# srvk/eesen

Hardware: AMD Instinct MI355X
Metric: CTC training frames/sec (whole node), 4x512 BiLSTM (higher is better)
Workload: dtype f32

## Files before the change

### eesen_amd/csrc/net.cpp

```cpp
#include "net.h"

#include <algorithm>
#include <cmath>
#include <cstdio>
#include <cstring>

namespace eesen {


int PhaseTimer::begin(hipStream_t st, int phase) {
  if (!on_) return -1;
  if (used_ == spans_.size()) spans_.emplace_back();
  spans_[used_].phase = phase;
  spans_[used_].a.record(st);
  return (int)used_++;
}
void PhaseTimer::end(hipStream_t st, int idx) {
  if (!on_ || idx < 0) return;
  spans_[idx].b.record(st);
}
void PhaseTimer::collect(float* out, int nphase) {
  for (int i = 0; i < nphase; ++i) out[i] = 0.f;
  for (size_t i = 0; i < used_; ++i) {
    spans_[i].b.wait();
// ... 615 lines not shown
      EESEN_REQUIRE((long)L.inj_fmask.size() == (long)net.rows * ldY, EESEN_ERR_INVALID, "injected forward mask has the wrong shape");
      EESEN_HIP_CHECK(hipMemcpyAsync(L.fmask.p, L.inj_fmask.data(), L.inj_fmask.size() * sizeof(float), hipMemcpyHostToDevice, net.st));
      EESEN_HIP_CHECK(hipStreamSynchronize(net.st));
    } else {
      dropout_mask(net.st, L.fmask.p, net.rows, ldY, ldY, fwd_p, net.drop_seed + (++net.drop_counter) * 0x632BE59BD9B4E019ull, fw_seq);
    }
    L.cur_fwd_drop = true;
  }
  L.inj_fmask.clear(); L.inj_rmask.clear(); L.inj_rmask_rows = 0; L.inj_coin = -1;
}

void Net::propagate(const float* in, int nrows, int ld, bool is_device) {
  EESEN_REQUIRE(finalized, EESEN_ERR_STATE, "net not finalized");
  EESEN_REQUIRE(S > 0, EESEN_ERR_STATE, "SetSeqLengths must precede Propagate");
  EESEN_REQUIRE(nrows > 0 && nrows % S == 0, EESEN_ERR_INVALID, "row count must be a positive multiple of the sequence count");
  const int D = layers[0].din, D4 = pad4(D);
  EESEN_REQUIRE(ld >= D, EESEN_ERR_INVALID, "input leading dimension smaller than InputDim");
  EESEN_HIP_CHECK(hipSetDevice(device));
  rows = nrows;
  T = rows / S;
  for (int v : lens) EESEN_REQUIRE(v <= T, EESEN_ERR_INVALID, "sequence length exceeds the number of frames");
  timer.reset();

  if (input.reserve((size_t)rows * D4) || D4 != D) EESEN_HIP_CHECK(hipMemsetAsync(input.p, 0, (size_t)rows * D4 * sizeof(float), st));
  if (is_device) {
    EESEN_HIP_CHECK(hipMemcpy2DAsync(input.p, (size_t)D4 * sizeof(float), in, (size_t)ld * sizeof(float), (size_t)D * sizeof(float), rows,
                                     hipMemcpyDeviceToDevice, st));
  } else {
    PinBuf& hs = in_stage[in_stage_idx++ & 1];
    const size_t bytes = (size_t)rows * D * sizeof(float);
    float* staged = static_cast<float*>(hs.reserve(bytes, bytes + bytes / 4));
    for (int r = 0; r < rows; ++r) std::memcpy(staged + (size_t)r * D, in + (size_t)r * ld, (size_t)D * sizeof(float));
    EESEN_HIP_CHECK(hipMemcpy2DAsync(input.p, (size_t)D4 * sizeof(float), staged, (size_t)D * sizeof(float), (size_t)D * sizeof(float), rows,
                                     hipMemcpyHostToDevice, st));
    hs.used(st);
  }
  forward_pass();
}

Net::FwdEarly Net::fwd_early(int li, const RecPlan& fp, int T) const {
  FwdEarly E;
  const Layer& L = layers[li];
  const Layer* nxt = li + 1 < (int)layers.size() ? &layers[li + 1] : nullptr;
  const int nd = L.ndir, ldY = nd * L.H;
  const long rows = (long)T * S;
  const bool pers = fp.kind != kRecNone;
  E.gate = pers && overlap && gate_fwd && !fwd_bf16 && !L.cur_fwd_drop && fp.units <= 8 && nxt && nxt->is_lstm() && T >= 2 && rows >= 128 &&
           fp.one_window &&
           (nxt->ndir * 4 * nxt->H) % 128 == 0 && ldY % 16 == 0 && nd * fp.seq_tiles * kShards <= 64;
  E.mile_step = (3 * T) / 4;
  E.mid = pers && overlap && tn.fwd_mid && !E.gate && !L.cur_fwd_drop && fp.leaves_room && nd == 2 && nxt && nxt->is_lstm() &&
          T >= 32 && E.mile_step + 1 < T && fp.one_window;
  if (E.mid) {
    E.r0 = ((T - 1 - E.mile_step) * S + 255) / 256 * 256;
    E.r1 = (E.mile_step + 1) * S / 256 * 256;
    if (E.r1 <= E.r0) E.r0 = E.r1 = 0;
  }
  return E;
}

bool Net::fwd_quad_rule(int li, const RecPlan& fp, int T, int r0, int r1, int steps[2]) const {
  steps[0] = steps[1] = -1;
  if (!tn.fwd_quad || li < 1 || r1 <= r0 || r0 <= 0 || (long)r1 >= (long)T * S) return false;
  const Layer& L = layers[li];
  if (L.ndir != 2 || fp.kind != kRecFwdBf || !fp.fn_guard || !fp.one_window || !fp.leaves_room || (4 * L.H) % 256 != 0) return false;
  steps[0] = std::min(r0 / S, T - 1 - (r1 - 1) / S);
  steps[1] = std::min(r1 / S, T - 1 - (r0 - 1) / S);
  return steps[0] >= 2 && steps[1] >= steps[0];
}

void Net::forward_pass() {
  const float* x = input.p;
  int ldx = pad4(layers[0].din);
  ++steps_since_clean;
  info_fwd_persistent = info_lstm_layers = info_fwd_bf16 = 0;
  dg_owner[0] = dg_owner[1] = -1;
  bool g_gated = false;
  int gated_rows = 0;
  int mid_r0 = 0, mid_r1 = 0;
  const bool half = gemm_mode() == 2;
  ensure_weight_amax();
  amx_valid = half;
  for (Layer& L : layers) {
    const int li_ = (int)(&L - layers.data());
    GemmBound x_amax, w_amax;
    if (half && L.trainable()) {
      if (x_is_bounded(li_)) x_amax = bound_one();
      else { measure(x, rows, L.din, ldx, L.bx.rows, L.bx.cols); x_amax = GemmBound{L.bx.rows.p, 1}; }
      w_amax = GemmBound{L.bw.rows.p, 1};
    }
    if (L.is_lstm()) {
      const int H = L.H, nd = L.ndir, ldY = nd * H, ldG = nd * 4 * H;
      L.G.reserve((size_t)rows * ldG);
      const size_t state = (size_t)(T + 2) * S * ldY;
      L.C.reserve(state);
      L.Y.reserve(state);
      if (persistent && H % 32 == 0) L.X.reserve((size_t)T * nd * ((S + 15) / 16) * (size_t)(H / 32) * 768);
      const size_t blk = (size_t)S * ldY * sizeof(float);
      EESEN_HIP_CHECK(hipMemsetAsync(L.C.p, 0, blk, st));
      EESEN_HIP_CHECK(hipMemsetAsync(L.Y.p, 0, blk, st));
      EESEN_HIP_CHECK(hipMemsetAsync(L.C.p + (size_t)(T + 1) * S * ldY, 0, blk, st));
      EESEN_HIP_CHECK(hipMemsetAsync(L.Y.p + (size_t)(T + 1) * S * ldY, 0, blk, st));
      prepare_dropout(*this, L);
      LstmLayerDev v = lstm_view(*this, L, T);
      const RecPlan fp = persistent ? lstm_fwd_plan(v) : RecPlan{};
      const bool pers = fp.kind != kRecNone;
      int quad_steps[2];
      const bool quad = !g_gated && fwd_quad_rule(li_, fp, T, mid_r0, mid_r1, quad_steps);
      if (quad) {
        unsigned* gw = mile.p + ((li_ - 1) & 1) * kMileRegion + kGuardWord;
        const int N4 = 4 * H;
        const float* Wx = params.p + L.p_off + L.off_wx;
        const float* bias = params.p + L.p_off + L.off_bias;
        GemmBound w_hi = w_amax;
        if (w_hi.p && w_hi.per_index) w_hi.p += N4;
        const int ti_ = timer.begin(st, 0);
        gemm_f32(st, true, true, mid_r0, N4, L.din, 1.f, x, ldx, Wx, pad4(L.din), 0.f, L.G.p, ldG, bias, nullptr, 0, 0, fwd_bf16, x_amax, w_amax);
        gemm_f32(st, true, true, rows - mid_r1, N4, L.din, 1.f, x + (size_t)mid_r1 * ldx, ldx, Wx + (size_t)N4 * pad4(L.din), pad4(L.din), 0.f,
                 L.G.p + (size_t)mid_r1 * ldG + N4, ldG, bias + N4, nullptr, 0, 0, fwd_bf16, x_amax, w_hi);
        timer.end(st, ti_);
        EESEN_HIP_CHECK(hipEventRecord(ev_quad_go, st));
        EESEN_HIP_CHECK(hipMemsetD32Async(reinterpret_cast<hipDeviceptr_t>(gw), 1, 1, st2));
        EESEN_HIP_CHECK(hipStreamWaitEvent(st2, ev_quad_go, 0));
        const int late_lds = tn.fwd_quad == 2 ? 64 : (tn.side_lds_kb >= 0 ? tn.side_lds_kb : (gemm_mode() >= 1 ? 48 : 32)) * 1024;
        const int tj_ = timer.begin(st2, 0);
        gemm_f32(st2, true, true, rows - mid_r1, N4, L.din, 1.f, x + (size_t)mid_r1 * ldx, ldx, Wx, pad4(L.din), 0.f, L.G.p + (size_t)mid_r1 * ldG, ldG,
                 bias, nullptr, 0, late_lds, fwd_bf16, x_amax, w_amax);
        gemm_f32(st2, true, true, mid_r0, N4, L.din, 1.f, x, ldx, Wx + (size_t)N4 * pad4(L.din), pad4(L.din), 0.f, L.G.p + N4, ldG, bias + N4,
                 nullptr, 0, late_lds, fwd_bf16, x_amax, w_hi);
        timer.end(st2, tj_);
        EESEN_HIP_CHECK(hipMemsetD32Async(reinterpret_cast<hipDeviceptr_t>(gw + 1), 1, 1, st2));
        EESEN_HIP_CHECK(hipEventRecord(ev_quad_done, st2));
        v.guard[0] = gw; v.guard_step[0] = quad_steps[0];
        v.guard[1] = gw + 1; v.guard_step[1] = quad_steps[1];
        mid_r0 = mid_r1 = 0;
      } else if (g_gated) {
        if (gated_rows < rows) {
          const int ti_ = timer.begin(st, 0);
          gemm_f32(st, true, true, rows - gated_rows, ldG, L.din, 1.f, x + (size_t)gated_rows * ldx, ldx, params.p + L.p_off + L.off_wx,
                   pad4(L.din), 0.f, L.G.p + (size_t)gated_rows * ldG, ldG, params.p + L.p_off + L.off_bias, nullptr, 0, 0, fwd_bf16, x_amax, w_amax);
          timer.end(st, ti_);
        }
        EESEN_HIP_CHECK(hipStreamWaitEvent(st, ev_gate_done, 0));
        g_gated = false;
      } else if (mid_r1 > mid_r0) {
        const int ti_ = timer.begin(st, 0);
        const int parts[2][2] = {{0, mid_r0}, {mid_r1, rows}};
        for (const auto& pr : parts)
          if (pr[1] > pr[0])
            gemm_f32(st, true, true, pr[1] - pr[0], ldG, L.din, 1.f, x + (size_t)pr[0] * ldx, ldx, params.p + L.p_off + L.off_wx, pad4(L.din),
                     0.f, L.G.p + (size_t)pr[0] * ldG, ldG, params.p + L.p_off + L.off_bias, nullptr, 0, 0, fwd_bf16, x_amax, w_amax);
        timer.end(st, ti_);
        EESEN_HIP_CHECK(hipStreamWaitEvent(st, ev_gate_done, 0));
        mid_r0 = mid_r1 = 0;
      } else {
        const int ti_ = timer.begin(st, 0);
        gemm_f32(st, true, true, rows, ldG, L.din, 1.f, x, ldx, params.p + L.p_off + L.off_wx, pad4(L.din), 0.f, L.G.p, ldG,
                 params.p + L.p_off + L.off_bias, nullptr, 0, 0, fwd_bf16, x_amax, w_amax);
        timer.end(st, ti_);
      }
      Layer* nxt = (&L - layers.data()) + 1 < (long)layers.size() ? &layers[(&L - layers.data()) + 1] : nullptr;
      const FwdEarly early = fwd_early(li_, fp, T);
      const bool plan_gate = early.gate;
      const int mile_step = early.mile_step;
      const bool plan_mid = early.mid;
      { const int ti_ = timer.begin(st, 1);
      v.poll_delay = delay_fwd;
      v.poll_raw = poll_raw;
      if (plan_mid) {
        mile.reserve(2 * kMileRegion);
        unsigned* region = mile.p + (li_ & 1) * kMileRegion;
        EESEN_HIP_CHECK(hipMemsetAsync(region, 0, kMileRegion * sizeof(unsigned), st));
        EESEN_HIP_CHECK(hipEventRecord(ev_gate_reset, st));
        v.milestone = region;
        v.milestone_step = mile_step;
      }
      if (pers) lstm_fwd_launch(st, fp, v, ctl.p, ctl.p + kCtlWords - 1, spin_limit, trace.p, plan_gate ? ev_gate_reset.get() : nullptr);
      else
        for (int step = 0; step < T; ++step) lstm_fwd_step(st, v, step);
      info_fwd_persistent += pers ? 1 : 0;
      info_fwd_bf16 += fp.bf16 ? 1 : 0;
      ++info_lstm_layers;
      check_launch("lstm_fwd");
      timer.end(st, ti_);
      if (quad) EESEN_HIP_CHECK(hipStreamWaitEvent(st, ev_quad_done, 0));
      if (pers && plan_gate) {
        const int ldG2 = nxt->ndir * 4 * nxt->H;
        nxt->G.reserve((size_t)rows * ldG2);
        EESEN_HIP_CHECK(hipStreamWaitEvent(st2, ev_gate_reset, 0));
        const int tj_ = timer.begin(st2, 0);
        GemmGate gate{ctl.p, ctl.p + kCtlWords - 1, nd, fp.seq_tiles, fp.grid[0], T, S, spin_limit};
        gated_rows = rows / 128 * 128;
        gemm_f32_nt_gated(st2, gated_rows, ldG2, ldY, L.Y.p + (size_t)S * ldY, ldY, params.p + nxt->p_off + nxt->off_wx, pad4(nxt->din),
                          nxt->G.p, ldG2, params.p + nxt->p_off + nxt->off_bias, gate, half ? bound_one() : GemmBound{}, half ? GemmBound{nxt->bw.rows.p, 1} : GemmBound{});
        timer.end(st2, tj_);
        EESEN_HIP_CHECK(hipEventRecord(ev_gate_done, st2));
        g_gated = true;
      }
      if (plan_mid) {
        EESEN_HIP_CHECK(hipMemsetD32Async(reinterpret_cast<hipDeviceptr_t>(v.milestone + 1), 1, 1, st));
        const int ldG2 = nxt->ndir * 4 * nxt->H;
        nxt->G.reserve((size_t)rows * ldG2);
        mid_r0 = early.r0;
        mid_r1 = early.r1;
      }
      if (plan_mid && mid_r1 > mid_r0) {
        const int ldG2 = nxt->ndir * 4 * nxt->H;
        EESEN_HIP_CHECK(hipStreamWaitEvent(st2, ev_gate_reset, 0));
        wait_for_word(st2, v.milestone + 1, 1u, ctl.p + kCtlWords - 1, 2.0 * std::max(1.0, T / 1000.0) * std::max(1.0, spin_limit / 400000.0));
        const int tj_ = timer.begin(st2, 0);
        gemm_f32(st2, true, true, mid_r1 - mid_r0, ldG2, nxt->din, 1.f, L.Y.p + (size_t)S * ldY + (size_t)mid_r0 * ldY, ldY,
                 params.p + nxt->p_off + nxt->off_wx, pad4(nxt->din), 0.f, nxt->G.p + (size_t)mid_r0 * ldG2, ldG2,
                 params.p + nxt->p_off + nxt->off_bias, nullptr, 0,  64, fwd_bf16,
                 half ? bound_one() : GemmBound{}, half ? GemmBound{nxt->bw.rows.p, 1} : GemmBound{});
        timer.end(st2, tj_);
        EESEN_HIP_CHECK(hipEventRecord(ev_gate_done, st2));
      } }
      if (L.cur_fwd_drop)
        mul_elements(st, L.Y.p + (size_t)S * ldY, ldY, L.fmask.p, ldY, L.Yd.p, ldY, rows, ldY);
      x = L.output(S);
      ldx = ldY;
    } else if (L.kind == EESEN_LAYER_AFFINE) {
      const int ldo = pad4(L.dout);
      if (L.out.reserve((size_t)rows * ldo)) EESEN_HIP_CHECK(hipMemsetAsync(L.out.p, 0, L.out.cap * sizeof(float), st));
      { const int ti_ = timer.begin(st, 2);
      gemm_f32(st, true, true, rows, L.dout, L.din, 1.f, x, ldx, params.p + L.p_off + L.off_w, pad4(L.din), 0.f, L.out.p, ldo,
               params.p + L.p_off + L.off_b, nullptr, 0, 0, fwd_bf16, x_amax, w_amax);
      timer.end(st, ti_); }
      x = L.out.p;
      ldx = ldo;
    } else if (L.is_activation()) {
      const int ldo = pad4(L.dout);
      if (L.out.reserve((size_t)rows * ldo)) EESEN_HIP_CHECK(hipMemsetAsync(L.out.p, 0, L.out.cap * sizeof(float), st));
      { const int ti_ = timer.begin(st, 2);
      activation_rows(st, L.kind == EESEN_LAYER_TANH, x, ldx, L.out.p, ldo, rows, L.dout);
      timer.end(st, ti_); }
      x = L.out.p;
      ldx = ldo;
    } else {
      const int ldo = pad4(L.dout);
      if (L.out.reserve((size_t)rows * ldo)) EESEN_HIP_CHECK(hipMemsetAsync(L.out.p, 0, L.out.cap * sizeof(float), st));
      { const int ti_ = timer.begin(st, 2);
      softmax_rows(st, x, ldx, L.out.p, ldo, rows, L.dout);
      timer.end(st, ti_); }
      x = L.out.p;
      ldx = ldo;
    }
  }
  out_ptr = x;
  out_cols = layers.back().dout;
  out_ld = ldx;
  if (const Layer& Lb = layers.back(); Lb.out_nb) {
    const int ldo = pad4(Lb.dout_f);
    if (out_f.reserve((size_t)rows * ldo) && ldo != Lb.dout_f) EESEN_HIP_CHECK(hipMemsetAsync(out_f.p, 0, out_f.cap * sizeof(float), st));
    for (int b = 0; b < Lb.out_nb; ++b) copy2d(st, x + (size_t)b * Lb.out_hi, ldx, out_f.p + (size_t)b * Lb.out_hf, ldo, rows, Lb.out_hf);
    out_ptr = out_f.p; out_cols = Lb.dout_f; out_ld = ldo;
  }
  propagated = true;
  if (persistent) arm_device_error_poll();
}

void Net::backpropagate(const float* out_diff, int ldd, float* in_diff, int ldi) {
  bucket_log.clear();
  deferred_buckets.clear();
  try {
    backpropagate_impl(out_diff, ldd, in_diff, ldi);
  } catch (...) {
    fail_step_buckets();
    throw;
  }
}

void Net::backpropagate_impl(const float* out_diff, int ldd, float* in_diff, int ldi) {
  EESEN_REQUIRE(propagated, EESEN_ERR_STATE, "Backpropagate needs a preceding Propagate");
  EESEN_HIP_CHECK(hipSetDevice(device));
  int maxdim = 0, max_g = 0, max_y = 0;
  size_t need_ws = 0;
  for (const Layer& L : layers) {
    maxdim = std::max(maxdim, std::max(pad4(L.din), pad4(L.dout)));
    if (L.is_lstm()) {
      max_g = std::max(max_g, L.ndir * 4 * L.H);
      max_y = std::max(max_y, L.ndir * L.H);
      need_ws = std::max(need_ws, lstm_bias_peep_ws_floats(T, S, L.H, L.ndir));
    }
    need_ws = std::max(need_ws, col_sums_ws_floats(rows, L.dout));
  }
  need_ws = std::max(need_ws, (size_t)16 << 20);
  ws.reserve(need_ws);
  ws_floats = need_ws;
  dA.reserve((size_t)rows * maxdim);
  dB.reserve((size_t)rows * maxdim);
  if (max_g) {
    DGb[0].reserve((size_t)rows * max_g);
    DGb[1].reserve((size_t)rows * max_g);
  }
  if (max_y) DCF.reserve((size_t)S * max_y);
  ws2.reserve(need_ws);
  int dg_slot = 0;
  dg_owner[0] = dg_owner[1] = -1;
  bool side_pending[2] = {false, false};
  deferred_buckets.clear();
  const std::vector<RecPlan> bwd = bwd_plans(T);
  const bool overlap = overlap_for_minibatch(bwd);
  exchange_deferred = comm && exchange_deferred_for_minibatch(bwd);
  bucket_log.clear();
  info_bwd_persistent = 0;
  live_valid = comm != nullptr;
  if (comm) {
    comm_check_alive(comm);
    EESEN_HIP_CHECK(hipMemsetD32Async(reinterpret_cast<hipDeviceptr_t>(fresh.p + P), 0x3f800000, 1, st));
  }

  const int Kout = layers.back().dout;
  float* d = dA.p;
  int ld_d = pad4(Kout);
  float* dn = dB.p;
  const bool half = gemm_mode() == 2;
  ensure_weight_amax();
  auto x_cols = [&](int li) -> GemmBound {
    if (!half || !amx_valid) return GemmBound{};
    return x_is_bounded(li) ? bound_one() : GemmBound{layers[li].bx.cols.p, 1};
  };
  if (const Layer& Lb = layers.back(); Lb.out_nb) {
    EESEN_HIP_CHECK(hipMemsetAsync(d, 0, (size_t)rows * ld_d * sizeof(float), st));
    for (int b = 0; b < Lb.out_nb; ++b) copy2d(st, out_diff + (size_t)b * Lb.out_hf, ldd, d + (size_t)b * Lb.out_hi, ld_d, rows, Lb.out_hf);
  } else {
    if (ld_d != Kout) EESEN_HIP_CHECK(hipMemsetAsync(d, 0, (size_t)rows * ld_d * sizeof(float), st));
    copy2d(st, out_diff, ldd, d, ld_d, rows, Kout);
  }

  for (int li = (int)layers.size() - 1; li >= 0; --li) {
    Layer& L = layers[li];
    const float* x;
    int ldx;
    if (li == 0) { x = input.p; ldx = pad4(L.din); }
    else {
      const Layer& Pv = layers[li - 1];
      if (Pv.is_lstm()) { ldx = Pv.ndir * Pv.H; x = Pv.output(S); }
      else { ldx = pad4(Pv.dout); x = Pv.out.p; }
    }
    const bool want_in = li > 0 || in_diff != nullptr;
    const int ld_n = pad4(L.din);
    float* fr = fresh.p + L.p_off;
    if (L.kind == EESEN_LAYER_SOFTMAX) {
      continue;
    } else if (L.is_activation()) {
      { const int ti_ = timer.begin(st, 4);
      activation_diff_rows(st, L.kind == EESEN_LAYER_TANH, L.out.p, pad4(L.dout), d, ld_d, rows, L.dout);
      timer.end(st, ti_); }
      continue;
    } else if (L.kind == EESEN_LAYER_AFFINE) {
      { const int ti_ = timer.begin(st, 4);
      if (half) measure(d, rows, L.dout, ld_d, L.bd.rows, L.bd.cols);
      if (want_in) {
        if (ld_n != L.din) EESEN_HIP_CHECK(hipMemsetAsync(dn, 0, (size_t)rows * ld_n * sizeof(float), st));
        gemm_f32(st, true, false, rows, L.din, L.dout, 1.f, d, ld_d, params.p + L.p_off + L.off_w, pad4(L.din), 0.f, dn, ld_n,
                 nullptr, nullptr, 0, 0, false, half ? GemmBound{L.bd.rows.p, 1} : GemmBound{}, half ? GemmBound{L.bw.cols.p, 1} : GemmBound{});
      }
      gemm_f32(st, false, false, L.dout, L.din, rows, 1.f, d, ld_d, x, ldx, 0.f, fr + L.off_w, pad4(L.din), nullptr, ws.p, ws_floats, 0, false,
               half ? GemmBound{L.bd.cols.p, 1} : GemmBound{}, x_cols(li));
      col_sums(st, d, rows, L.dout, ld_d, fr + L.off_b, ws.p, ws_floats);
      timer.end(st, ti_); }
      bucket_allreduce(li, st);
    } else {
      const int H = L.H, nd = L.ndir, ldG = nd * 4 * H, ldY = nd * H;
      LstmLayerDev v = lstm_view(*this, L, T);
      v.poll_delay = overlap ? delay_bwd_side : delay_bwd;
      v.poll_raw = poll_raw;
      const RecPlan& bp = bwd[li];
      if (bp.need_px) { bwd_px.reserve(bp.need_px); v.PX = bwd_px.p; v.px_floats = bwd_px.cap; }
      if (bp.need_dgh) {
        bwd_dgh.reserve((size_t)rows * ldG);
        bwd_ex.reserve(bp.need_ex);
        v.DGH = reinterpret_cast<unsigned char*>(bwd_dgh.p);
        v.EX = bwd_ex.p;
      }
      EESEN_REQUIRE(in_train || !L.has_dropout(), EESEN_ERR_STATE, "Can't backpropagate a dropout layer in test mode (bilstm-parallel-layer.h:425)");
      if (L.cur_fwd_drop) mul_elements(st, d, ld_d, L.fmask.p, ldY, d, ld_d, rows, ldY);
      float* DGl = DGb[dg_slot].p;
      dg_owner[dg_slot] = li;
      if (side_pending[dg_slot]) {
        EESEN_HIP_CHECK(hipStreamWaitEvent(st, ev_grad[dg_slot], 0));
        side_pending[dg_slot] = false;
      }
      { const int ti_ = timer.begin(st, 3);
      if (bp.kind != kRecNone) {
        lstm_bwd_launch(st, bp, v, d, ld_d, DGl, ctl.p + kCtlHalf, ctl.p + kCtlWords - 1, spin_limit, trace.p ? trace.p + 640 : nullptr);
        ++info_bwd_persistent;
      } else
        for (int step = 0; step < T; ++step) lstm_bwd_step(st, v, step, d, ld_d, DGl, DCF.p);
      check_launch("lstm_bwd");
      timer.end(st, ti_); }
      if (half) { const int ti_ = timer.begin(st, 4); measure(DGl, rows, ldG, ldG, L.bd.rows, L.bd.cols); timer.end(st, ti_); }
      EESEN_HIP_CHECK(hipEventRecord(ev_rec, st));
      if (want_in) {
        const int ti_ = timer.begin(st, 4);
        if (ld_n != L.din) EESEN_HIP_CHECK(hipMemsetAsync(dn, 0, (size_t)rows * ld_n * sizeof(float), st));
        gemm_f32(st, true, false, rows, L.din, ldG, 1.f, DGl, ldG, params.p + L.p_off + L.off_wx, pad4(L.din), 0.f, dn, ld_n,
                 nullptr, nullptr, 0, 0, false, half ? GemmBound{L.bd.rows.p, 1} : GemmBound{}, half ? GemmBound{L.bw.cols.p, 1} : GemmBound{});
        timer.end(st, ti_);
        EESEN_HIP_CHECK(hipEventRecord(ev_rec, st));
      }
      hipStream_t sg = overlap ? st2 : st;
      const int side_lds_env = (tn.side_lds_kb >= 0 ? tn.side_lds_kb : (gemm_mode() >= 1 ? 48 : 32)) * 1024;
      bool lstm_below = false;
      for (int lj = 0; lj < li; ++lj) lstm_below |= layers[lj].is_lstm();
      const int side_lds = overlap && lstm_below ? side_lds_env : 0;
      if (overlap) EESEN_HIP_CHECK(hipStreamWaitEvent(st2, ev_rec, 0));
      { const int ti_ = timer.begin(sg, 4);
      gemm_f32(sg, false, false, ldG, L.din, rows, 1.f, DGl, ldG, x, ldx, 0.f, fr + L.off_wx, pad4(L.din), nullptr, ws2.p, need_ws, side_lds, false,
               half ? GemmBound{L.bd.cols.p, 1} : GemmBound{}, x_cols(li));
      for (int dir = 0; dir < nd; ++dir)
        gemm_f32(sg, false, false, 4 * H, H, rows, 1.f, DGl + (size_t)dir * 4 * H, ldG,
                 L.Y.p + (size_t)(dir == 0 ? 0 : 2 * S) * ldY + (size_t)dir * H, ldY, 0.f,
                 fr + L.off_wm + (size_t)dir * 4 * H * H, H, nullptr, ws2.p, need_ws, side_lds, false,
                 half ? GemmBound{L.bd.cols.p + (size_t)dir * 4 * H, 1} : GemmBound{}, half ? bound_one() : GemmBound{});
      lstm_bias_peep_grads(sg, v, DGl, fr + L.off_bias, fr + L.off_peep, ws2.p, need_ws);
      timer.end(sg, ti_); }
      bucket_allreduce(li, sg);
      if (overlap) {
        EESEN_HIP_CHECK(hipEventRecord(ev_grad[dg_slot], st2));
        side_pending[dg_slot] = true;
      }
      dg_slot ^= 1;
    }
    if (want_in) {
      std::swap(d, dn);
      ld_d = ld_n;
    }
  }
  if (in_diff) copy2d(st, d, ld_d, in_diff, ldi, rows, layers[0].din);
  flush_deferred_buckets();
  for (int k = 0; k < 2; ++k)
    if (side_pending[k]) EESEN_HIP_CHECK(hipStreamWaitEvent(st, ev_grad[k], 0));
}

std::vector<RecPlan> Net::bwd_plans(int T) const {
  std::vector<RecPlan> plans(layers.size());
  for (size_t li = 0; li < layers.size(); ++li)
    if (persistent && layers[li].is_lstm()) plans[li] = lstm_bwd_plan(lstm_view(*this, layers[li], T));
  return plans;
}
bool Net::overlap_for_minibatch(const std::vector<RecPlan>& bwd) const {
  bool ov = overlap;
  if (ov && tn.overlap < 0 && persistent)
    for (size_t li = 0; li < layers.size(); ++li)
      if (const Layer& L = layers[li]; L.is_lstm() && L.H > 320 && L.H <= 512 && S > 32 && !bwd[li].light) ov = false;
  return ov;
}
bool Net::exchange_deferred_for_minibatch(const std::vector<RecPlan>& bwd) const {
  if (tn.comm_defer >= 0) return tn.comm_defer != 0;
  if (!persistent) return false;
  for (const RecPlan& bp : bwd)
    if (bp.kind != kRecNone && bp.free_vgprs < kRcclVgprsPerSimdLane) return true;
  return false;
}

std::string Net::plan_string() const {
  EESEN_REQUIRE(finalized, EESEN_ERR_STATE, "net not finalized");
  EESEN_REQUIRE(S > 0, EESEN_ERR_STATE, "call eesen_net_set_seq_lengths first: the plan depends on the minibatch shape");
  EESEN_HIP_CHECK(hipSetDevice(device));
  int T = this->T;
  if (!propagated) { T = 0; for (int v : lens) T = std::max(T, v); }
  auto one = [](const RecPlan& P) {
    char b[512];
    if (P.kind == kRecNone) { snprintf(b, sizeof(b), "{\"kernel\": \"per-step kernels (lstm.hip)\", \"persistent\": false}"); return std::string(b); }
    snprintf(b, sizeof(b), "{\"kernel\": \"%s\", \"persistent\": true, \"sequences_per_workgroup\": %d, \"units_per_workgroup\": %d, \"grid\": [%d, %d, %d], "
             "\"workgroups\": %d, \"workgroups_per_cu\": %d, \"launches\": %d, \"vgprs\": %d, \"lds_bytes\": %d, \"free_vgprs_per_simd_lane\": %d}",
             P.kernel, P.seq_tile, P.units, P.grid[0], P.grid[1], P.grid[2], P.wgs, P.wgs_per_cu, P.windows, P.vgprs, P.lds, P.free_vgprs);
    return std::string(b);
  };
  const std::vector<RecPlan> bwd = bwd_plans(T);
  std::string o = "{\"T\": " + std::to_string(T) + ", \"S\": " + std::to_string(S) + ", \"persistent\": " + (persistent ? "true" : "false") + ", \"layers\": [";
  bool first = true;
  FwdEarly below;
  for (size_t li = 0; li < layers.size(); ++li) {
    const Layer& L = layers[li];
    if (!L.is_lstm()) { below = FwdEarly{}; continue; }
    const RecPlan fp = persistent && T >= 1 ? lstm_fwd_plan(lstm_view(*this, L, T)) : RecPlan{}, &bp = bwd[li];
    int qs[2];
    const char* sched = below.gate ? "gated under the recurrence below"
                        : below.r1 > below.r0 ? (fwd_quad_rule((int)li, fp, T, below.r0, below.r1, qs) ? "middle under the recurrence below, needed quadrants, recurrence, late quadrants beside it"
                                                                                                  : "middle under the recurrence below, both ends, recurrence")
                                              : "whole, recurrence";
    const bool lstm_below = li > 0 && layers[li - 1].is_lstm();
    o += std::string(first ? "" : ", ") + "{\"layer\": " + std::to_string(li) + ", \"cells\": " + std::to_string(L.H) + ", \"directions\": " + std::to_string(L.ndir) +
         ", \"forward\": " + one(fp) + ", \"backward\": " + one(bp) + (lstm_below ? std::string(", \"input_gemm\": \"") + sched + "\"" : std::string()) + "}";
    below = T >= 1 ? fwd_early((int)li, fp, T) : FwdEarly{};
    first = false;
  }
  const bool ov = overlap_for_minibatch(bwd);
  o += std::string("], \"weight_gradient_gemms\": \"") + (ov ? "side stream, under the next-lower recurrence" : "main stream, serial") + "\"";
  o += std::string(", \"gemm_arithmetic\": \"") + (gemm_mode() == 2 ? "two fp16 planes, three products (fp32-class)" : gemm_mode() == 1 ? "3-way bf16 split (fp32-class)" : "f32-input MFMA") + "\"";
  o += std::string(", \"exchange\": ") + (comm ? (exchange_deferred_for_minibatch(bwd) ? "\"deferred: every bucket behind the backward pass's last recurrence\""
                                                                                      : "\"overlapped: each bucket as soon as its layer's gradients are enqueued\"") : "null");
  o += std::string(", \"exchange_rule\": \"") + (tn.comm_defer >= 0 ? "EESEN_COMM_DEFER" : "auto: deferred when a persistent backward grid leaves < 256 registers per SIMD lane") + "\"";
  o += ", \"gpu_share\": " + std::to_string(gpu_share_value()) + "}";
  return o;
}

void Net::update() {
  EESEN_REQUIRE(finalized, EESEN_ERR_STATE, "net not finalized");
  EESEN_HIP_CHECK(hipSetDevice(device));
  const unsigned* skip = persistent && !grads_sanitized ? ctl.p + kCtlWords - 1 : nullptr;
  const float* live = comm && live_valid ? fresh.p + P : nullptr;
  comm_check_alive(comm);
  { const int ti_ = timer.begin(st, 5);
  for (int li = (int)layers.size() - 1; li >= 0; --li) {
    Layer& L = layers[li];
    if (L.p_n) {
      if (comm && li < (int)bucket_pending.size() && bucket_pending[li]) {
        const int tw_ = timer.begin(st, 7);
        EESEN_HIP_CHECK(hipStreamWaitEvent(st, ev_bucket[li], 0));
        timer.end(st, tw_);
        bucket_pending[li] = 0;
      }
      if (rule == 0) {
        sgd_update(st, params.p + L.p_off, corr.p + L.p_off, fresh.p + L.p_off, (long)L.p_n, mmt, lr * L.coef, L.max_grad, skip, live);
      } else {
        init_accu();
        adaptive_update(st, params.p + L.p_off, corr.p + L.p_off, fresh.p + L.p_off, accu.p + L.p_off, (long)L.p_n, mmt, lr,
                        L.max_grad, ada_eps, rms_rho, rms_one_minus_rho, rule == 2, skip, live);
      }
    }
  }
  refresh_derived();
  timer.end(st, ti_); }
  grads_sanitized = false;
  live_valid = false;
  if (persistent) arm_device_error_poll();
}

}
```

### eesen_amd/csrc/net.h

```cpp
#pragma once
#include <string>
#include <vector>

#include "ctc_layout.h"
#include "kernels.h"
#include "lex.h"
#include "lm.h"
#include "tuning.h"

namespace eesen {

inline int pad4(int x) { return (x + 3) & ~3; }
constexpr size_t kCtlWords = 2 * kCtlHalf + 32;

struct Layer {
  int kind = 0, din = 0, dout = 0;
  float coef = 1.f, max_grad = 0.f;
  size_t p_off = 0, p_n = 0;
  int H = 0, ndir = 0;
  int din_f = 0, dout_f = 0, Hf = 0;
  int in_nb = 0, in_hf = 0, in_hi = 0, out_nb = 0, out_hf = 0, out_hi = 0;
  int in_col(int d) const { return in_nb ? (d / in_hf) * in_hi + d % in_hf : d; }
  size_t off_wx = 0, off_bias = 0, off_wm = 0, off_peep = 0;
  DevBuf<float> WmT;
  DevBuf<float> G, C, Y;
  DevBuf<float> X;
  size_t off_w = 0, off_b = 0;
  DevBuf<float> out;
  struct Bounds { DevBuf<float> rows, cols; } bw, bx, bd;
  float drop[9] = {0, 0, 0, 0, 0, 0, 0, 0, 0};
  bool has_dropout() const { return drop[0] > 0.f || drop[5] != 0.f || drop[6] != 0.f; }
  DevBuf<float> fmask;
  DevBuf<float> rmask;
  DevBuf<float> Yd;
  bool cur_fwd_drop = false;
  int cur_drop_mode = 0;
  bool cur_twiddle_coin = false;
  std::vector<float> inj_fmask, inj_rmask;
  int inj_rmask_rows = 0, inj_coin = -1;
  const float* output(int S) const { return cur_fwd_drop ? Yd.p : Y.p + (size_t)S * ndir * H; }
  bool is_lstm() const { return kind == EESEN_LAYER_LSTM_PARALLEL || kind == EESEN_LAYER_BILSTM_PARALLEL; }
  bool nonparallel = false;
  bool is_activation() const { return kind == EESEN_LAYER_SIGMOID || kind == EESEN_LAYER_TANH; }
  bool trainable() const { return is_lstm() || kind == EESEN_LAYER_AFFINE; }
  long file_params() const;
  const char* marker() const;
};

class PhaseTimer {
 public:
  void enable(bool on) { on_ = on; }
  bool enabled() const { return on_; }
  void set_accumulate(bool a) { accumulate_ = a; used_ = 0; }
  void reset() { if (!accumulate_) used_ = 0; }
  int begin(hipStream_t st, int phase);
  void end(hipStream_t st, int idx);
  void collect(float* out, int nphase);
  int spans(int* phases, float* secs, int cap);
 private:
  struct Span { DevEvent a{true}, b{true}; int phase = 0; };
  std::vector<Span> spans_;
  size_t used_ = 0;
  bool on_ = false, accumulate_ = false;
};

class PhaseClock {
 public:
  static constexpr int kMaxPhases = 3;
  void set_mode(bool accumulate) { spans_.enable(accumulate); spans_.set_accumulate(accumulate); }
  void mark(hipStream_t st, int phase);
  void stop(hipStream_t st);
  void read(float* out, int nphase);
 private:
  DevEvent ev_[kMaxPhases + 1] = {DevEvent(true), DevEvent(true), DevEvent(true), DevEvent(true)};
  PhaseTimer spans_;
  int phase_ = 0, span_ = -1;
};

struct Comm;
void comm_check_alive(const Comm* c);
constexpr size_t kLiveWords = 4;
constexpr int kRcclVgprsPerSimdLane = 256;

struct StatGuard {
  const unsigned* word = nullptr;
  struct Net* net = nullptr;
  long dropped = 0;
  hipStream_t st = nullptr;
  StatGuard() = default;
  StatGuard(const StatGuard&) = delete;
  StatGuard& operator=(const StatGuard&) = delete;
  ~StatGuard() { unhook(); }
  void hook(struct Net* n, int device, hipStream_t stream, const char* entry_point);
  void unhook();
  void note_dropped(const char* what);
  void* read_back(PinBuf& pin, const void* dev, size_t bytes, hipStream_t stream, bool guarded = true);
  static bool raised(const void* host, size_t bytes);
};

struct Net {
  int device = 0;
  hipStream_t st = nullptr;
  std::vector<Layer> layers;
  bool finalized = false;
  size_t P = 0;
  DevBuf<float> params, corr, fresh;
  float lr = 0.f, mmt = 0.f;
  int rule = 0;
  float ada_eps = 1e-6f, rms_rho = 0.9f, rms_one_minus_rho = 0.1f;
  DevBuf<float> accu;
  bool accu_init = false;
  void init_accu();
  void set_accu(const float* host, long n);
  std::vector<int> lens;
  DevBuf<int> lens_d;
  int T = 0, S = 0, rows = 0;
  bool propagated = false;
  DevBuf<float> input;
  PinBuf in_stage[2];
  unsigned in_stage_idx = 0;
  const float* out_ptr = nullptr;
  int out_cols = 0, out_ld = 0;
  DevBuf<float> out_f;
  DevBuf<float> DGb[2], DCF, dA, dB, ws, ws2;
  DevBuf<float> bwd_px;
  DevBuf<float> bwd_dgh, bwd_ex;
  DevStream st2;
  DevEvent ev_rec, ev_grad[2];
  bool overlap = true;
  DevEvent ev_gate_reset, ev_gate_done;
  DevBuf<unsigned> mile;
  static constexpr int kMileRegion = 64, kGuardWord = 32;
  DevEvent ev_quad_go, ev_quad_done;
  struct FwdEarly { bool gate = false, mid = false; int mile_step = 0, r0 = 0, r1 = 0; };
  FwdEarly fwd_early(int li, const RecPlan& fp, int T) const;
  bool fwd_quad_rule(int li, const RecPlan& fp, int T, int r0, int r1, int steps[2]) const;
  bool gate_fwd = true;
  bool fwd_bf16 = false;
  bool fwd_bf16_rec = false;
  int info_fwd_bf16 = 0;
  DevBuf<unsigned> ctl;
  Tuning tn;
  int persistent = 1;
  int info_fwd_persistent = 0, info_bwd_persistent = 0, info_lstm_layers = 0;
  int spin_limit = 400000;
  float flight_ns = 0.f;
  int delay_fwd = 61, delay_bwd = 43, delay_bwd_side = 64, poll_raw = 0;
  int recoveries = 0;
  DevBuf<unsigned long long> trace;
  void check_device_error(bool consumer);
  int steps_since_clean = 0;
  PinBuf lens_pin, err_pin;
  bool err_armed = false;
  void poll_device_error();
  void arm_device_error_poll();
  bool in_train = true;
  unsigned long long drop_seed = 777, drop_counter = 0;
  void set_train_mode(bool train) { in_train = train; }
  int dg_owner[2] = {-1, -1};
  void debug_layer_buffer(int layer, int which, float* host, long cap_floats, int* rows_out, int* cols_out);
  void set_layer_dropout(int layer, const float* nine);
  void get_layer_dropout(int layer, float* nine) const;
  void set_dropout_masks(int layer, const float* fwd, long fwd_n, const float* rec, int rec_rows, long rec_n, int coin);
  void get_dropout_masks(int layer, float* fwd_host, float* rec_host, int* info4);
  size_t ws_floats = 0;
  DevBuf<float> amax, amax_ws;
  bool wamax_valid = false, wm_valid = false;
  bool amx_valid = false;
  float* am_wm(int li) { return amax.p + 1 + li; }
  GemmBound bound_one() const { return GemmBound{amax.p, 0}; }
  bool x_is_bounded(int li) const;
  void measure(const float* P, long rows, int cols, int ld, DevBuf<float>& out_rows, DevBuf<float>& out_cols);
  void ensure_weight_amax();
  PhaseTimer timer;
  Comm* comm = nullptr;
  std::vector<DevEvent> ev_ready, ev_bucket;
  std::vector<char> bucket_pending;
  std::vector<int> deferred_buckets;
  bool exchange_deferred = false;
  std::vector<RecPlan> bwd_plans(int T) const;
  bool overlap_for_minibatch(const std::vector<RecPlan>& bwd) const;
  bool exchange_deferred_for_minibatch(const std::vector<RecPlan>& bwd) const;
  std::string plan_string() const;
  DevEvent ev_bwd_done;
  void issue_bucket(int li);
  void fail_step_buckets() noexcept;
  void flush_deferred_buckets();
  std::vector<StatGuard*> guards;
  bool grads_sanitized = false;
  bool live_valid = false;
  std::vector<int> bucket_log;
  PinBuf live_pin;
  void set_comm(Comm* c);
  int top_trainable() const;
  int live_ranks();
  void bucket_allreduce(int li, hipStream_t producer);
  void wait_buckets_host();
  void backpropagate_zero();
  void allreduce_grads(Comm* c);

  Net(int device, void* stream);
  ~Net();
  void add_layer(int kind, int din, int dout, float coef, float max_grad);
  void finalize();
  long num_params() const;
  void set_params(const float* host, long n);
  void get_flat(const DevBuf<float>& buf, float* host, long n);
  void set_seq_lengths(const int* lens, int S);
  void propagate(const float* in, int rows, int ld, bool is_device);
  void forward_pass();
  void backpropagate(const float* out_diff, int ldd, float* in_diff, int ldi);
  void backpropagate_impl(const float* out_diff, int ldd, float* in_diff, int ldi);
  void update();
  void refresh_derived();
  int tensor_moments(int which, int layer, double* out6_host, int cap_tensors);
  void read(const std::string& path);
  void write(const std::string& path, bool binary);
  void sync();
};

inline void* loss_slot(PinBuf& pin, size_t bytes) { return pin.reserve(bytes, std::max<size_t>(bytes * 2, 4096)); }

struct StageSlots {
  PinBuf slot[2];
  unsigned idx = 0;
  template <class Fill> void upload(hipStream_t st, int* dst, size_t n, Fill&& fill) {
    PinBuf& sp = slot[idx++ & 1];
    int* pinned = static_cast<int*>(loss_slot(sp, n * sizeof(int)));
    fill(pinned);
    EESEN_HIP_CHECK(hipMemcpyAsync(dst, pinned, n * sizeof(int), hipMemcpyHostToDevice, st));
    sp.used(st);
  }
};

void check_shape(const int* frame_num_utt, int S, int rows, int K, int ld, int min_K);

struct Ctc {
  int device = 0;
  hipStream_t st = nullptr;
  DevBuf<float> logp, alpha, beta, pzx_d;
  DevBuf<int> labx, ids_d, ali_d;
  std::vector<int> last_lens;
  int last_T = 0, last_S = 0, last_Lpad = 0, last_Lprime = 0;
  int sweep_waves = 0;
  double obj_sum = 0;
  long sequences = 0, frames = 0, err_tokens = 0, ref_tokens = 0;
  PhaseClock clock;
  PhaseClock align_clock;
  PinBuf align_pin;
  DevBuf<float> dec_f;
  DevBuf<int> dec_i, dec_trie, dec_out;
  PhaseClock decode_clock;
  PinBuf decode_pin;
  DecodeLayout dec;
  std::vector<int> dec_lens;
  int dec_space = -1;
  int dec_tokens() const { return dec.mode == kDecodeWords ? 2 : dec_space >= 0 ? 1 : 0; }
  std::vector<int> dec_word, dec_word_len;
  DevBuf<int> stamp_i;
  PhaseClock stamp_clock;
  PinBuf stamp_pin;
  int stamp_group = 0;
  DevBuf<int> score_i;
  PhaseClock rescore_clock;
  double rescore_host_s = 0;
  PinBuf score_pin;
  int dec_V = 0;
  DevBuf<int> ed_i;
  PinBuf ed_pin;
  DevEvent mev[2] = {DevEvent(true), DevEvent(true)};
  double mbr_t[3] = {0, 0, 0};
  bool mbr_accumulate = false;
  DevBuf<int> lm_i;
  DevBuf<float> lm_f;
  LmTables lm_tab{};
  unsigned long long lm_serial = 0;
  DevBuf<int> lex_i;
  LexTables lex_tab{};
  WordLexTables word_tab{};
  unsigned long long lex_serial = 0;
  int lm_lookahead = 0;
  DevBuf<float> la_f;
  unsigned long long la_lex_serial = 0, la_lm_serial = 0;
  StageSlots stage;
  struct PendingPzx { PinBuf pin; int S = 0; long nframes = 0; bool active = false; } ppzx[2];
  struct PendingErr { PinBuf pin, probs; int S = 0, K = 0, rows = 0; bool active = false, with_probs = false; std::vector<int> frames, ids, off; } perr[2];
  StatGuard guard;
  std::string seq_out;
  unsigned ppzx_idx = 0, perr_idx = 0;
  void flush_pzx(PendingPzx& q);
  void flush_err(PendingErr& q, int* num_err, int* num_ref);
  void flush();

  Ctc(int device, void* stream);
  ~Ctc();
  void eval_parallel(const int* frame_num_utt, int S, const float* net_out, int rows, int K, int ld, const int* label_ids,
                     const int* label_off, float* diff, int ldd, float* pzx_host);
  void error_rate_mseq(const int* frame_num_utt, int S, const float* net_out, int rows, int K, int ld,
                       const int* label_ids, const int* label_off, int* num_err, int* num_ref);
  void get_alpha_beta(float* alpha_host, float* beta_host, int* Lprime);
  void set_profiling(int mode);
  void phase_times(float* out3) { clock.read(out3, 3); }
  void align_parallel(const int* frame_num_utt, int S, const float* scores, int rows, int K, int ld, bool is_log, const int* label_ids,
                      const int* label_off, int* ali_host, int* pos_host, float* score_host);
  void align_times(float* out3) { align_clock.read(out3, 3); }
  void decode_parallel(const int* frame_num_utt, int S, const float* scores, int rows, int K, int ld, bool is_log, int beam, int max_classes,
                       int nbest, int* hyp_host, int* hyp_len_host, float* score_host);
  void decode_parallel_lm(const int* frame_num_utt, int S, const float* scores, int rows, int K, int ld, bool is_log, int beam, int max_classes,
                          int nbest, const TokenLm* lm, float lm_weight, float insertion_bonus, bool use_eos, int* hyp_host, int* hyp_len_host,
                          float* score_host, float* lm_score_host);
  void decode_parallel_lex(const int* frame_num_utt, int S, const float* scores, int rows, int K, int ld, bool is_log, int beam, int max_classes,
                           int nbest, const Lexicon* lex, const TokenLm* lm, float lm_weight, float word_bonus, bool use_eos, int* hyp_host,
                           int* hyp_len_host, float* score_host, float* lm_score_host, int* word_host, int* word_len_host);
  void decode_parallel_words(const int* frame_num_utt, int S, const float* scores, int rows, int K, int ld, bool is_log, int beam, int max_classes,
                             int nbest, const Lexicon* lex, const TokenLm* lm, float lm_weight, float word_bonus, bool use_eos, int* hyp_host,
                             int* hyp_len_host, float* score_host, float* lm_score_host, int* word_host, int* word_len_host, int* word_end_host);
  void decode_times(float* out3) { decode_clock.read(out3, 3); }
  void decode_stamps(const int* frame_num_utt, int S, const float* scores, int rows, int K, int ld, bool is_log, double conf_scale,
                     int* lstart_host, int* lend_host, int* wstart_host, int* wend_host, float* wconf_host, float* path_score_host);
  void stamp_times(float* out3) { stamp_clock.read(out3, 3); }
  void score_parallel(const int* frame_num_utt, int S, const float* scores, int rows, int K, int ld, bool is_log, const int* hyp_off,
                      const int* label_off, const int* label_ids, float* score_host);
  void decode_rescore(const int* frame_num_utt, int S, const float* scores, int rows, int K, int ld, bool is_log, const TokenLm* lm,
                      float lm_weight, float bonus, bool use_eos, float* am_host, float* lm_host, float* total_host, int* order_host);
  void rescore_times(float* out3) { rescore_clock.read(out3, 2); out3[2] = (float)rescore_host_s; }
  void edit_distance_parallel(int G, const int* seq_off, const int* tok_off, const int* tok_ids, const int* ref_off, const int* ref_ids,
                              int* pair_host, int* ref_dist_host);
  void decode_mbr(int S, int level, double scale, const float* total_host, const int* ref_off, const int* ref_ids, int* dist_host,
                  int* ref_dist_host, double* post_host, double* risk_host, int* order_host);
  void mbr_times(float* out3);
  void get_decode_candidates(int* ids_host, float* scores_host, float* blank_host, int* Cc);
 private:
  struct Lattices { const int *labx, *lens, *lablens; int Lpad, Lprime; };
  Lattices upload_lattices(const int* frame_num_utt, int S, const int* label_ids, const int* label_off);
  void decode_batch(const int* frame_num_utt, int S, const float* scores, int rows, int K, int ld, bool is_log, int beam, int max_classes,
                    int nbest, const Lexicon* lex, const TokenLm* lm, float lm_weight, float bonus, bool use_eos, int* hyp_host, int* hyp_len_host,
                    float* score_host, float* lm_score_host, int* word_host, int* word_len_host, int* word_end_host);
  void upload_lm(const TokenLm& lm);
  void upload_lex(const Lexicon& lex);
  const float* upload_lookahead(const Lexicon* lex, const TokenLm* lm);
  const int* ed_run(const int* tok_h, size_t n_tok, const int* dev_tok, const std::vector<int>& jobs, size_t n_same, int max_len, bool* bad);
};

void word_confidence(int n, const double* scores, const int* word_len, const int* word_ids, const int* wstart, const int* wend, int stride,
                     double conf_scale, double* conf_out);

int edit_distance(const int* ref, int nr, const int* hyp, int nh);

struct CeLoss {
  int device = 0;
  hipStream_t st = nullptr;
  DevBuf<int> tg;
  DevBuf<CeSums> part, res;
  StageSlots stage;
  struct Pending { PinBuf pin; int S = 0; long rows = 0; bool active = false; } pend[2];
  unsigned pend_idx = 0;
  double obj = 0, obj_progress = 0;
  long correct = 0, frames = 0, sequences = 0, correct_progress = 0, frames_progress = 0, sequences_progress = 0;
  int report_step = 100;
  std::vector<std::string> progress;
  StatGuard guard;
  PhaseClock clock;

  CeLoss(int device, void* stream);
  ~CeLoss();
  void fold(Pending& q, double* obj_out);
  void flush();
  void eval_parallel(const int* frame_num_utt, int S, const float* net_out, int rows, int K, int ld, const int* targets,
                     float* diff, int ldd, double* obj_host);
  std::string report();
  void phase_times(float* out1) { clock.read(out1, 1); }
};

}
```

### eesen_amd/csrc/tuning.h

```cpp
#pragma once
#include <cstddef>
#include <cstdlib>

namespace eesen {

constexpr size_t kStampDeltaBytes = (size_t)1 << 30;

struct Tuning {
  int persistent = 1;
  int overlap = -1, gate_fwd = -1, side_lds_kb = -1;
  int spin_limit = 400000;
  bool spin_limit_set = false;
  int bwd_q4 = 1, bwd_q4_st8 = 1, fwd_narrow2 = 1, fwd_t16_small = 1, bwd_ksplit = 1, fwd_mux = 1, bwd_mux = 1, xcd_map = 1, fwd_mid = 1, fwd_quad = 1, fwd_split = 1, fwd_f16 = 1, bwd_f16 = 1;
  int comm_defer = -1;
  int trace = 0;
  bool print_flight = false;
  const char* poll_ns = nullptr;

  static Tuning from_env() {
    Tuning t;
    auto num = [](const char* name, int dflt) {
      const char* e = getenv(name);
      return e && *e ? atoi(e) : dflt;
    };
    t.persistent = num("EESEN_PERSISTENT", 1);
    t.overlap = num("EESEN_OVERLAP", -1);
    t.gate_fwd = num("EESEN_GATE_FWD", -1);
    t.fwd_mid = num("EESEN_FWD_MID", 1);
    t.fwd_quad = num("EESEN_FWD_QUAD", 1);
    t.side_lds_kb = num("EESEN_SIDE_LDS_KB", -1);
    t.spin_limit_set = getenv("EESEN_SPIN_LIMIT") != nullptr;
    t.spin_limit = num("EESEN_SPIN_LIMIT", 400000);
    t.bwd_q4 = num("EESEN_BWD_Q4", 1);
    t.bwd_q4_st8 = num("EESEN_BWD_Q4_ST8", 1);
    t.fwd_narrow2 = num("EESEN_FWD_NARROW2", 1);
    t.fwd_t16_small = num("EESEN_FWD_T16_SMALL", 1);
    t.bwd_ksplit = num("EESEN_BWD_KSPLIT", 1);
    t.fwd_mux = num("EESEN_FWD_MUX", 1);
    t.bwd_mux = num("EESEN_BWD_MUX", 1);
    t.fwd_split = num("EESEN_FWD_SPLIT", 1);
    t.fwd_f16 = num("EESEN_FWD_F16", 1);
    t.bwd_f16 = num("EESEN_BWD_F16", 1);
    t.xcd_map = num("EESEN_XCD_MAP", 1);
    t.comm_defer = num("EESEN_COMM_DEFER", -1);
    t.trace = num("EESEN_TRACE", 0);
    t.print_flight = getenv("EESEN_PRINT_FLIGHT") != nullptr;
    t.poll_ns = getenv("EESEN_POLL_NS");
    return t;
  }
};

}
```

Baseline: 1.028 million.

## Spread backward weight-gradient GEMMs across main and side streams

Adds a bwd_spread bitmask (default 7) that moves more backward weight-gradient work onto the side stream. Affine-layer weight and bias gradients now run on the side stream when LSTM layers sit below, guarded by a new event before the next layer reuses the dn buffer. For the bottom LSTM layer, the Wx gradient and bias/peephole gradients go to the main stream while the recurrent Wm gradient runs on the side stream. The LSTM poll delay now depends on whether side-stream LSTM grads are actually in flight. The aim is to overlap more gradient GEMMs with the recurrent backward kernels, at the cost of extra event syncs and side-stream contention with the persistent kernels.

```diff
diff --git a/eesen_amd/csrc/net.cpp b/eesen_amd/csrc/net.cpp
--- a/eesen_amd/csrc/net.cpp
+++ b/eesen_amd/csrc/net.cpp
@@ -941,6 +941,14 @@
   deferred_buckets.clear();
   const std::vector<RecPlan> bwd = bwd_plans(T);
   const bool overlap = overlap_for_minibatch(bwd);
+  const int spread = overlap ? tn.bwd_spread : 0;
+  const int side_lds_env = (tn.side_lds_kb >= 0 ? tn.side_lds_kb : (gemm_mode() >= 1 ? 48 : 32)) * 1024;
+  bool aff_pending = false;
+  bool side_lstm_grads = false;
+  auto dn_free = [&] {
+    if (aff_pending) EESEN_HIP_CHECK(hipStreamWaitEvent(st, ev_aff, 0));
+    aff_pending = false;
+  };
   exchange_deferred = comm && exchange_deferred_for_minibatch(bwd);
   bucket_log.clear();
   info_bwd_persistent = 0;
@@ -981,6 +989,8 @@
     const bool want_in = li > 0 || in_diff != nullptr;
     const int ld_n = pad4(L.din);
     float* fr = fresh.p + L.p_off;
+    bool lstm_below = false;
+    for (int lj = 0; lj < li; ++lj) lstm_below |= layers[lj].is_lstm();
     if (L.kind == EESEN_LAYER_SOFTMAX) {
       continue;
     } else if (L.is_activation()) {
@@ -989,22 +999,36 @@
       timer.end(st, ti_); }
       continue;
     } else if (L.kind == EESEN_LAYER_AFFINE) {
-      { const int ti_ = timer.begin(st, 4);
+      const bool aff_side = (spread & 1) && lstm_below;
+      hipStream_t sa = aff_side ? st2.s : st;
+      float* wsa = aff_side ? ws2.p : ws.p;
+      { int ti_ = timer.begin(st, 4);
       if (half) measure(d, rows, L.dout, ld_d, L.bd.rows, L.bd.cols);
       if (want_in) {
+        dn_free();
         if (ld_n != L.din) EESEN_HIP_CHECK(hipMemsetAsync(dn, 0, (size_t)rows * ld_n * sizeof(float), st));
         gemm_f32(st, true, false, rows, L.din, L.dout, 1.f, d, ld_d, params.p + L.p_off + L.off_w, pad4(L.din), 0.f, dn, ld_n,
                  nullptr, nullptr, 0, 0, false, half ? GemmBound{L.bd.rows.p, 1} : GemmBound{}, half ? GemmBound{L.bw.cols.p, 1} : GemmBound{});
       }
-      gemm_f32(st, false, false, L.dout, L.din, rows, 1.f, d, ld_d, x, ldx, 0.f, fr + L.off_w, pad4(L.din), nullptr, ws.p, ws_floats, 0, false,
-               half ? GemmBound{L.bd.cols.p, 1} : GemmBound{}, x_cols(li));
-      col_sums(st, d, rows, L.dout, ld_d, fr + L.off_b, ws.p, ws_floats);
-      timer.end(st, ti_); }
-      bucket_allreduce(li, st);
+      if (aff_side) {
+        timer.end(st, ti_);
+        EESEN_HIP_CHECK(hipEventRecord(ev_rec, st));
+        EESEN_HIP_CHECK(hipStreamWaitEvent(sa, ev_rec, 0));
+        ti_ = timer.begin(sa, 4);
+      }
+      gemm_f32(sa, false, false, L.dout, L.din, rows, 1.f, d, ld_d, x, ldx, 0.f, fr + L.off_w, pad4(L.din), nullptr, wsa, ws_floats,
+               aff_side ? side_lds_env : 0, false, half ? GemmBound{L.bd.cols.p, 1} : GemmBound{}, x_cols(li));
+      col_sums(sa, d, rows, L.dout, ld_d, fr + L.off_b, wsa, ws_floats);
+      timer.end(sa, ti_); }
+      bucket_allreduce(li, sa);
+      if (aff_side) {
+        EESEN_HIP_CHECK(hipEventRecord(ev_aff, sa));
+        aff_pending = true;
+      }
     } else {
       const int H = L.H, nd = L.ndir, ldG = nd * 4 * H, ldY = nd * H;
       LstmLayerDev v = lstm_view(*this, L, T);
-      v.poll_delay = overlap ? delay_bwd_side : delay_bwd;
+      v.poll_delay = ((spread & 4) ? side_lstm_grads : overlap) ? delay_bwd_side : delay_bwd;
       v.poll_raw = poll_raw;
       const RecPlan& bp = bwd[li];
       if (bp.need_px) { bwd_px.reserve(bp.need_px); v.PX = bwd_px.p; v.px_floats = bwd_px.cap; }
@@ -1034,6 +1058,7 @@
       EESEN_HIP_CHECK(hipEventRecord(ev_rec, st));
       if (want_in) {
         const int ti_ = timer.begin(st, 4);
+        dn_free();
         if (ld_n != L.din) EESEN_HIP_CHECK(hipMemsetAsync(dn, 0, (size_t)rows * ld_n * sizeof(float), st));
         gemm_f32(st, true, false, rows, L.din, ldG, 1.f, DGl, ldG, params.p + L.p_off + L.off_wx, pad4(L.din), 0.f, dn, ld_n,
                  nullptr, nullptr, 0, 0, false, half ? GemmBound{L.bd.rows.p, 1} : GemmBound{}, half ? GemmBound{L.bw.cols.p, 1} : GemmBound{});
@@ -1041,25 +1066,41 @@
         EESEN_HIP_CHECK(hipEventRecord(ev_rec, st));
       }
       hipStream_t sg = overlap ? st2 : st;
-      const int side_lds_env = (tn.side_lds_kb >= 0 ? tn.side_lds_kb : (gemm_mode() >= 1 ? 48 : 32)) * 1024;
-      bool lstm_below = false;
-      for (int lj = 0; lj < li; ++lj) lstm_below |= layers[lj].is_lstm();
       const int side_lds = overlap && lstm_below ? side_lds_env : 0;
       if (overlap) EESEN_HIP_CHECK(hipStreamWaitEvent(st2, ev_rec, 0));
-      { const int ti_ = timer.begin(sg, 4);
-      gemm_f32(sg, false, false, ldG, L.din, rows, 1.f, DGl, ldG, x, ldx, 0.f, fr + L.off_wx, pad4(L.din), nullptr, ws2.p, need_ws, side_lds, false,
-               half ? GemmBound{L.bd.cols.p, 1} : GemmBound{}, x_cols(li));
-      for (int dir = 0; dir < nd; ++dir)
-        gemm_f32(sg, false, false, 4 * H, H, rows, 1.f, DGl + (size_t)dir * 4 * H, ldG,
-                 L.Y.p + (size_t)(dir == 0 ? 0 : 2 * S) * ldY + (size_t)dir * H, ldY, 0.f,
-                 fr + L.off_wm + (size_t)dir * 4 * H * H, H, nullptr, ws2.p, need_ws, side_lds, false,
-                 half ? GemmBound{L.bd.cols.p + (size_t)dir * 4 * H, 1} : GemmBound{}, half ? bound_one() : GemmBound{});
-      lstm_bias_peep_grads(sg, v, DGl, fr + L.off_bias, fr + L.off_peep, ws2.p, need_ws);
-      timer.end(sg, ti_); }
+      auto grad_wx = [&](hipStream_t s, float* w) {
+        gemm_f32(s, false, false, ldG, L.din, rows, 1.f, DGl, ldG, x, ldx, 0.f, fr + L.off_wx, pad4(L.din), nullptr, w, need_ws, side_lds, false,
+                 half ? GemmBound{L.bd.cols.p, 1} : GemmBound{}, x_cols(li));
+      };
+      auto grad_wm = [&](hipStream_t s, float* w) {
+        for (int dir = 0; dir < nd; ++dir)
+          gemm_f32(s, false, false, 4 * H, H, rows, 1.f, DGl + (size_t)dir * 4 * H, ldG,
+                   L.Y.p + (size_t)(dir == 0 ? 0 : 2 * S) * ldY + (size_t)dir * H, ldY, 0.f,
+                   fr + L.off_wm + (size_t)dir * 4 * H * H, H, nullptr, w, need_ws, side_lds, false,
+                   half ? GemmBound{L.bd.cols.p + (size_t)dir * 4 * H, 1} : GemmBound{}, half ? bound_one() : GemmBound{});
+      };
+      if ((spread & 2) && !lstm_below) {
+        { const int ti_ = timer.begin(sg, 4);
+        grad_wm(sg, ws2.p);
+        timer.end(sg, ti_); }
+        { const int ti_ = timer.begin(st, 4);
+        grad_wx(st, ws.p);
+        lstm_bias_peep_grads(st, v, DGl, fr + L.off_bias, fr + L.off_peep, ws.p, need_ws);
+        timer.end(st, ti_); }
+        EESEN_HIP_CHECK(hipEventRecord(ev_half, st));
+        EESEN_HIP_CHECK(hipStreamWaitEvent(sg, ev_half, 0));
+      } else {
+        const int ti_ = timer.begin(sg, 4);
+        grad_wx(sg, ws2.p);
+        grad_wm(sg, ws2.p);
+        lstm_bias_peep_grads(sg, v, DGl, fr + L.off_bias, fr + L.off_peep, ws2.p, need_ws);
+        timer.end(sg, ti_);
+      }
       bucket_allreduce(li, sg);
       if (overlap) {
         EESEN_HIP_CHECK(hipEventRecord(ev_grad[dg_slot], st2));
         side_pending[dg_slot] = true;
+        side_lstm_grads = true;
       }
       dg_slot ^= 1;
     }
@@ -1072,6 +1113,7 @@
   flush_deferred_buckets();
   for (int k = 0; k < 2; ++k)
     if (side_pending[k]) EESEN_HIP_CHECK(hipStreamWaitEvent(st, ev_grad[k], 0));
+  dn_free();
 }
 
 std::vector<RecPlan> Net::bwd_plans(int T) const {
diff --git a/eesen_amd/csrc/net.h b/eesen_amd/csrc/net.h
--- a/eesen_amd/csrc/net.h
+++ b/eesen_amd/csrc/net.h
@@ -127,6 +127,8 @@
   DevBuf<float> bwd_dgh, bwd_ex;
   DevStream st2;
   DevEvent ev_rec, ev_grad[2];
+  DevEvent ev_aff;
+  DevEvent ev_half;
   bool overlap = true;
   DevEvent ev_gate_reset, ev_gate_done;
   DevBuf<unsigned> mile;
diff --git a/eesen_amd/csrc/tuning.h b/eesen_amd/csrc/tuning.h
--- a/eesen_amd/csrc/tuning.h
+++ b/eesen_amd/csrc/tuning.h
@@ -12,6 +12,7 @@
   int spin_limit = 400000;
   bool spin_limit_set = false;
   int bwd_q4 = 1, bwd_q4_st8 = 1, fwd_narrow2 = 1, fwd_t16_small = 1, bwd_ksplit = 1, fwd_mux = 1, bwd_mux = 1, xcd_map = 1, fwd_mid = 1, fwd_quad = 1, fwd_split = 1, fwd_f16 = 1, bwd_f16 = 1;
+  int bwd_spread = 7;
   int comm_defer = -1;
   int trace = 0;
   bool print_flight = false;
@@ -29,6 +30,7 @@
     t.fwd_mid = num("EESEN_FWD_MID", 1);
     t.fwd_quad = num("EESEN_FWD_QUAD", 1);
     t.side_lds_kb = num("EESEN_SIDE_LDS_KB", -1);
+    t.bwd_spread = num("EESEN_BWD_SPREAD", 7);
     t.spin_limit_set = getenv("EESEN_SPIN_LIMIT") != nullptr;
     t.spin_limit = num("EESEN_SPIN_LIMIT", 400000);
     t.bwd_q4 = num("EESEN_BWD_Q4", 1);
```

New measurement: 1.037 million, median of 6. No clear change (+0.9%).
